# han0110/learn-fhe

Hardware: AMD Instinct MI355X
Metric: NTTs/sec at N=2^14 q~60-bit (higher is better)
Workload: dtype u64

## Files before the change

learn-fhe_amd/csrc/arith.hpp:

```cpp
#pragma once
#include <type_traits>

#include "dev_arith.hpp"

namespace fhe {

#define FHE_GLOBAL __attribute__((address_space(1)))
template <class T>
__device__ __forceinline__ const FHE_GLOBAL T *as_global(const T *p) {
    return (const FHE_GLOBAL T *)p;
}
#define FHE_CONST __attribute__((address_space(4)))
template <class T>
__device__ __forceinline__ const FHE_CONST T *as_const(const T *p) {
    return (const FHE_CONST T *)p;
}

#define FHE_HEADER_KERNEL static __attribute__((unused)) __global__

template <int I, int END, typename F>
__device__ __forceinline__ void static_for(F &&f) {
    if constexpr (I < END) {
        f(std::integral_constant<int, I>{});
        static_for<I + 1, END>(f);
// ... 162 lines not shown
    static __device__ __forceinline__ TwRaw fetch(const K &k, int idx) {
        const FHE_CONST PmRaw *p = (INV ? k.twi : k.tw) + idx;
        TwRaw r;
        r.x = p->x; r.y = p->y;
        return r;
    }
    static __device__ __forceinline__ TwReg prep(const TwRaw &r) { return PmTw{r.x, r.x << (63 - B), r.y}; }
    static __host__ __device__ __forceinline__ PmTw split(u64 w) {
        PmTw t;
        t.wl = (unsigned)(w & ((u64(1) << (B - 31)) - 1));
        t.wlp = t.wl << (63 - B);
        t.wh = (unsigned)(w >> (B - 31));
        return t;
    }
    static __device__ __forceinline__ K make(const ModDesc &D, int log_n_total, int pb, int prefix) {
        K k;
        k.m.q = D.q; k.m.q2 = 2 * D.q; k.m.q4 = 4 * D.q;
        k.m.c = D.pm_c; k.m.c2 = 2 * D.pm_c;
        k.tw = (const FHE_CONST PmRaw *)D.tww; k.twi = (const FHE_CONST PmRaw *)D.twwi;
        k.ninv = split(pb ? 1 : D.ninv[log_n_total]);
        k.ninv_w = split(D.ninv_w[log_n_total]);
        k.pb = pb; k.prefix = prefix;
        return k;
    }
    static __device__ __forceinline__ u64 fold1(u64 x, const PmK &m) {
        const unsigned hi = (unsigned)(x >> 32), h = hi >> (B - 32);
        const u64 base = ((u64)(hi & (unsigned)(MASK >> 32)) << 32) | (unsigned)x;
        return (u64)h * m.c + base;
    }
    static __device__ __forceinline__ u64 mulvar(u64 x, u64 y, const K &k) { return pm_mul<B>(x, split(y), k.m); }
    static __device__ __forceinline__ void ct(u64 &X, u64 &Y, const TwReg &w, const K &k) {
        const u64 t = pm_mul<B>(Y, w, k.m);
        const u64 x = X;
        X = x + t;
        Y = x - t + k.m.q2;
    }
    template <int PH>
    static __device__ __forceinline__ void gs(u64 &X, u64 &Y, const TwReg &w, const K &k) {
        const u64 s = X + Y;
        const u64 d = X - Y + (PH ? k.m.q4 : k.m.q2);
        X = s;
        Y = pm_mul<B>(d, w, k.m);
    }
    static constexpr bool GS_FOLDS = true;
    static constexpr int GS_SPAN = 0;
    template <int PH = 1>
    static __device__ __forceinline__ void gs_last_scaled(u64 &X, u64 &Y, const K &k) {
        const u64 s = X + Y, d = X - Y + k.m.q4;
        X = csub(pm_mul<B>(s, k.ninv, k.m), k.m.q);
        Y = csub(pm_mul<B>(d, k.ninv_w, k.m), k.m.q);
    }
    template <int PH = 1>
    static __device__ __forceinline__ void gs_last_plain(u64 &X, u64 &Y, const PmTw &w, const K &k) {
        const u64 s = X + Y, d = X - Y + k.m.q4;
        X = csub(fold1(s, k.m), k.m.q);
        Y = csub(pm_mul<B>(d, w, k.m), k.m.q);
    }
    static constexpr int CT_LAYERS = ((1 << (63 - B)) + 1) / 2 > 64 ? 64 : ((1 << (63 - B)) + 1) / 2;
    static constexpr bool PASS_FOLD = true;
    static __device__ constexpr bool ct_fold_at(int) { return false; }
    static __device__ __forceinline__ u64 gs_fold(u64 x, const K &k) { return fold1(x, k.m); }
    static __device__ __forceinline__ u64 fold(u64 x, const K &k) { return fold1(x, k.m); }
    static __device__ __forceinline__ u64 canon_fwd(u64 x, const K &k) { return csub(fold1(x, k.m), k.m.q); }
    static __device__ __forceinline__ u64 finish_inv(u64 x, const K &k) { return csub(pm_mul<B>(x, k.ninv, k.m), k.m.q); }
    static constexpr int MAC_TERMS = B <= 54 ? 32 : B == 55 ? 16 : B == 56 ? 8 : 3;
    struct MacAcc { u64 v, u; };
    static __device__ __forceinline__ MacAcc mac_zero() { return MacAcc{0, 0}; }
    static __device__ __forceinline__ u64 mac_in(u64 x, const K &) { return x; }
    static __device__ __forceinline__ MacAcc mac(MacAcc acc, u64 xin, u64 kval, int term, const K &k, const Barrett &) {
        const unsigned wl = (unsigned)kval;
        const PmTw w{wl, wl << (63 - B), (unsigned)(kval >> 32)};
        u64 v, u;
        pm_mul_vu<B>(xin, w, v, u);
        acc.v += v; acc.u += u;
        if ((term % MAC_TERMS) == MAC_TERMS - 1) acc = MacAcc{pm_reduce_vu<B>(acc.v, acc.u, k.m), 0};
        return acc;
    }
    static __device__ __forceinline__ u64 mac_finish(MacAcc acc, const K &k) { return pm_reduce_vu<B>(acc.v, acc.u, k.m); }
};

struct DsK {
    u64 q, q2, q4;
    unsigned c, c2, pw;
};

template <int B>
struct ArithDS {
    typedef u64 Elem;
    static constexpr u64 MASK = (u64(1) << B) - 1;
    static constexpr int SPLIT = B - 31;
    typedef uint4 TwRaw;
    typedef uint4 TwReg;
    struct K {
        DsK m;
        const FHE_CONST uint4 *tw, *twi;
        uint4 ninv, ninv_w;
        int pb, prefix;
        const FHE_CONST uint4 *tw3i;
        unsigned tw3_stride;
    };
    static constexpr int PREFETCH = 4;
    static __host__ __device__ __forceinline__ uint4 split(u64 w, u64 q) {
        const u64 w1 = (u64)((((unsigned __int128)w) << 32) % q);
        const u64 lo = (u64(1) << SPLIT) - 1;
        return uint4{(unsigned)(w & lo), (unsigned)(w >> SPLIT), (unsigned)(w1 & lo), (unsigned)(w1 >> SPLIT)};
    }
    template <bool INV>
    static __device__ __forceinline__ TwRaw fetch(const K &k, int idx) {
        const FHE_CONST uint4 *p = (INV ? k.twi : k.tw) + idx;
        TwRaw r;
        r.x = p->x; r.y = p->y; r.z = p->z; r.w = p->w;
        return r;
    }
    static __device__ __forceinline__ TwReg prep(const TwRaw &r) { return r; }
    static __device__ __forceinline__ K make(const ModDesc &D, int log_n_total, int pb, int prefix) {
        K k;
        k.m.q = D.q; k.m.q2 = 2 * D.q; k.m.q4 = 4 * D.q;
        k.m.c = D.pm_c; k.m.c2 = 2 * D.pm_c; k.m.pw = D.ds_pow;
        k.tw = as_const(D.twd); k.twi = as_const(D.twdi);
        k.ninv = pb ? D.ds_one : D.ds_ninv[log_n_total];
        k.ninv_w = D.ds_ninv_w[log_n_total];
        k.pb = pb; k.prefix = prefix;
        k.tw3i = as_const(D.twd3i); k.tw3_stride = D.twd3_stride;
        return k;
    }
    static __device__ __forceinline__ u64 mul_raw(u64 y, const uint4 &w, const DsK &m) {
        const unsigned y0 = (unsigned)y, y1 = (unsigned)(y >> 32);
        const u64 s1 = (u64)w.y * y0 + (u64)w.w * y1;
        const u64 s0 = (u64)w.x * y0 + (u64)w.z * y1;
        const u64 v = (u64)(unsigned)s1 * m.pw + s0;
        return (u64)(unsigned)(s1 >> 32) * m.c2 + v;
    }
    static __device__ __forceinline__ u64 fold1(u64 x, const DsK &m) {
        const unsigned hi = (unsigned)(x >> 32), h = hi >> (B - 32);
        const u64 base = ((u64)(hi & (unsigned)(MASK >> 32)) << 32) | (unsigned)x;
        return (u64)h * m.c + base;
    }
    static __device__ __forceinline__ u64 mul(u64 y, const uint4 &w, const DsK &m) { return fold1(mul_raw(y, w, m), m); }
    static __device__ __forceinline__ u64 mulvar(u64 x, u64 y, const K &k) {
        return pm_mul<B>(x, ArithPM<B>::split(y), PmK{k.m.q, k.m.q2, k.m.q4, k.m.c, k.m.c2});
    }
    static __device__ __forceinline__ void ct(u64 &X, u64 &Y, const TwReg &w, const K &k) {
        const u64 t = mul(Y, w, k.m);
        const u64 x = X;
        X = x + t;
        Y = x + k.m.q2 - t;
    }
    static constexpr int CT_LAYERS = 64;
    static constexpr bool PASS_FOLD = false;
    static constexpr int CT_SPAN = B >= 64 - 2 ? 1 : (((1 << (64 - B)) - 2) / 2 > 64 ? 64 : ((1 << (64 - B)) - 2) / 2);
    static __device__ constexpr bool ct_fold_at(int layer) { return layer > 0 && layer % CT_SPAN == 0; }
    template <int PH>
    static __device__ __forceinline__ void gs(u64 &X, u64 &Y, const TwReg &w, const K &k) {
        static_assert(PH < 64 - B - 1, "sums overflow");
        const u64 s = X + Y;
        const u64 d = X + (k.m.q2 << PH) - Y;
        X = s;
        Y = mul(d, w, k.m);
    }
    static constexpr bool GS_FOLDS = true;
    static constexpr int GS_SPAN = 64 - B - 1 > 8 ? 8 : 64 - B - 1;
    template <int PH = 1>
    static __device__ __forceinline__ void gs_last_scaled(u64 &X, u64 &Y, const K &k) {
        const u64 s = X + Y, d = X + (k.m.q2 << PH) - Y;
        X = csub(mul(s, k.ninv, k.m), k.m.q);
        Y = csub(mul(d, k.ninv_w, k.m), k.m.q);
    }
    template <int PH = 1>
    static __device__ __forceinline__ void gs_last_plain(u64 &X, u64 &Y, const TwReg &w, const K &k) {
        const u64 s = X + Y, d = X + (k.m.q2 << PH) - Y;
        X = csub(fold1(s, k.m), k.m.q);
        Y = csub(mul(d, w, k.m), k.m.q);
    }
    static __device__ __forceinline__ u64 gs_fold(u64 x, const K &k) { return fold1(x, k.m); }
    static __device__ __forceinline__ u64 fold(u64 x, const K &k) { return fold1(x, k.m); }
    static __device__ __forceinline__ u64 canon_fwd(u64 x, const K &k) { return csub(fold1(x, k.m), k.m.q); }
    static __device__ __forceinline__ u64 finish_inv(u64 x, const K &k) { return csub(mul(x, k.ninv, k.m), k.m.q); }
    typedef typename ArithPM<B>::MacAcc MacAcc;
    static constexpr int MAC_TERMS = ArithPM<B>::MAC_TERMS;
    static __device__ __forceinline__ PmK pmk(const K &k) { return PmK{k.m.q, k.m.q2, k.m.q4, k.m.c, k.m.c2}; }
    static __device__ __forceinline__ MacAcc mac_zero() { return MacAcc{0, 0}; }
    static __device__ __forceinline__ u64 mac_in(u64 x, const K &) { return x; }
    static __device__ __forceinline__ MacAcc mac(MacAcc acc, u64 xin, u64 kval, int term, const K &k, const Barrett &) {
        const unsigned wl = (unsigned)kval;
        const PmTw w{wl, wl << (63 - B), (unsigned)(kval >> 32)};
        u64 v, u;
        pm_mul_vu<B>(xin, w, v, u);
        acc.v += v; acc.u += u;
        if ((term % MAC_TERMS) == MAC_TERMS - 1) acc = MacAcc{pm_reduce_vu<B>(acc.v, acc.u, pmk(k)), 0};
        return acc;
    }
    static __device__ __forceinline__ u64 mac_finish(MacAcc acc, const K &k) { return pm_reduce_vu<B>(acc.v, acc.u, pmk(k)); }
};

#define FHE_SCHED_FENCE() asm volatile("" ::: "memory")

template <int L0_, int R_, int l_, int REP0_, int NREP_, int STRIDE_, bool SHARED_, int REP_SHIFT_ = 0>
struct Unit {
    static constexpr int L0 = L0_, R = R_, l = l_, REP0 = REP0_, NREP = NREP_, STRIDE = STRIDE_, REP_SHIFT = REP_SHIFT_;
    static constexpr bool SHARED = SHARED_;
    static constexpr int NT = (SHARED_ ? 1 : NREP_) << l_;
    static constexpr int half = 1 << (R_ - 1 - l_);
};

#ifdef FHE_LAB_ABLATE
template <class A, class = void> struct tw_skip_mask { static constexpr unsigned value = 0; };
template <class A> struct tw_skip_mask<A, decltype((void)A::SKIP_MASK)> { static constexpr unsigned value = A::SKIP_MASK; };
#endif

template <class A, bool INV, class U, int NTW>
__device__ __forceinline__ void tw_load(typename A::TwRaw (&raw)[NTW], int top, const typename A::K &k) {
    static_assert(U::NT <= NTW, "twiddle buffer too small for this unit");
#pragma unroll
    for (int rr = 0; rr < (U::SHARED ? 1 : U::NREP); ++rr)
#pragma unroll
        for (int b = 0; b < (1 << U::l); ++b) {
            const int tp = U::SHARED ? top : (top | ((U::REP0 + rr) << U::REP_SHIFT));
            const int idx = (1 << (U::L0 + U::l + k.pb)) + ((((k.prefix << U::L0) | tp)) << U::l) + b;
#ifdef FHE_LAB_ABLATE
            if constexpr ((tw_skip_mask<A>::value >> (U::L0 + U::l)) & 1) { raw[(rr << U::l) | b] = A::fake(k, idx); continue; }
#endif
            raw[(rr << U::l) | b] = A::template fetch<INV>(k, idx);
        }
}

template <class A, class U, int NTW, int E>
__device__ __forceinline__ void ct_apply(typename A::Elem (&x)[E], const typename A::TwRaw (&raw)[NTW], const typename A::K &k) {
    if constexpr ((U::l > 0 && U::l % A::CT_LAYERS == 0) || A::ct_fold_at(U::L0 + U::l)) {
#pragma unroll
        for (int rr = 0; rr < U::NREP; ++rr)
#pragma unroll
            for (int r = 0; r < (1 << U::R); ++r) x[(U::REP0 + rr) * U::STRIDE + r] = A::fold(x[(U::REP0 + rr) * U::STRIDE + r], k);
    }
    if constexpr (U::SHARED) {
#pragma unroll
        for (int b = 0; b < (1 << U::l); ++b) {
            const typename A::TwReg w = A::prep(raw[b]);
#pragma unroll
            for (int rr = 0; rr < U::NREP; ++rr)
#pragma unroll
                for (int j = 0; j < U::half; ++j) {
                    const int o = (U::REP0 + rr) * U::STRIDE + b * 2 * U::half + j;
                    A::ct(x[o], x[o + U::half], w, k);
                }
        }
    } else {
#pragma unroll
        for (int rr = 0; rr < U::NREP; ++rr)
#pragma unroll
            for (int b = 0; b < (1 << U::l); ++b) {
                const typename A::TwReg w = A::prep(raw[(rr << U::l) | b]);
#pragma unroll
                for (int j = 0; j < U::half; ++j) {
                    const int o = (U::REP0 + rr) * U::STRIDE + b * 2 * U::half + j;
                    A::ct(x[o], x[o + U::half], w, k);
                }
            }
    }
}

template <class A, class U, int GSTEP = -1, int NTW, int E>
__device__ __forceinline__ void gs_apply(typename A::Elem (&x)[E], const typename A::TwRaw (&raw)[NTW], const typename A::K &k) {
    constexpr bool GLOBAL = GSTEP >= 0 && A::GS_SPAN > 0;
    constexpr int step = U::R - 1 - U::l, PH = GLOBAL ? GSTEP % (A::GS_SPAN > 0 ? A::GS_SPAN : 1) : (step & 1);
    constexpr bool FOLD = A::GS_FOLDS && (GLOBAL ? PH == A::GS_SPAN - 1 : (PH == 1 || step == U::R - 1));
    static_for<0, (U::SHARED ? (1 << U::l) : U::NREP)>([&](auto oc) {
        constexpr int outer = decltype(oc)::value;
        static_for<0, (U::SHARED ? U::NREP : (1 << U::l))>([&](auto ic) {
            constexpr int inner = decltype(ic)::value;
            constexpr int b = U::SHARED ? outer : inner, rr = U::SHARED ? inner : outer;
            const typename A::TwReg w = A::prep(raw[U::SHARED ? b : ((rr << U::l) | b)]);
#pragma unroll
            for (int j = 0; j < U::half; ++j) {
                const int o = (U::REP0 + rr) * U::STRIDE + b * 2 * U::half + j;
                A::template gs<PH>(x[o], x[o + U::half], w, k);
                if constexpr (FOLD) x[o] = A::gs_fold(x[o], k);
            }
        });
    });
}

template <class A, int L0, int R, int OFF, int E>
__device__ __forceinline__ void ct_net(typename A::Elem (&x)[E], int top, const typename A::K &k) {
    static_for<0, R>([&](auto lc) {
        constexpr int l = decltype(lc)::value;
        typedef Unit<L0, R, l, 1, 1, OFF, true> U;
        if constexpr (l > 0) FHE_SCHED_FENCE();
        typename A::TwRaw raw[1 << l];
        tw_load<A, false, U>(raw, top, k);
        ct_apply<A, U>(x, raw, k);
    });
}

template <class A, int L0, int R, int OFF, int E>
__device__ __forceinline__ void gs_net(typename A::Elem (&x)[E], int top, const typename A::K &k) {
    static_for<0, R>([&](auto sc) {
        constexpr int l = R - 1 - decltype(sc)::value;
        typedef Unit<L0, R, l, 1, 1, OFF, true> U;
        if constexpr (l < R - 1) FHE_SCHED_FENCE();
        typename A::TwRaw raw[1 << l];
        tw_load<A, true, U>(raw, top, k);
        gs_apply<A, U>(x, raw, k);
    });
}

}
```

learn-fhe_amd/csrc/ntt14w.hpp:

```cpp
#pragma once
#include <type_traits>
#include "ntt_kernels.hpp"

namespace fhe {
namespace w14 {

constexpr int WSLOTS = 1088;
template <int R0> constexpr int threads() { return 64 << R0; }
template <int R0> constexpr size_t lds_bytes() { return (size_t(1) << R0) * WSLOTS * 8; }
constexpr int THREADS = threads<3>();
constexpr size_t LDS_BYTES = lds_bytes<3>();

__device__ __forceinline__ void wave_sync() {
    __builtin_amdgcn_wave_barrier();
    asm volatile("" ::: "memory");
}
#ifndef W14_XCHG_PRIO
#define W14_XCHG_PRIO 0
#endif
#if W14_XCHG_PRIO
#define W14_PRIO_UP() __builtin_amdgcn_s_setprio(3)
#define W14_PRIO_DOWN() __builtin_amdgcn_s_setprio(0)
#else
#define W14_PRIO_UP()
#define W14_PRIO_DOWN()
#endif

template <class A, class = void> struct w14_old_deal { static constexpr bool value = false; };
template <class A> struct w14_old_deal<A, decltype((void)A::W14_OLD_DEAL)> { static constexpr bool value = true; };
template <class A, int R0>
__device__ __host__ constexpr bool w14_pairs() {
    return R0 <= 3 && !w14_old_deal<A>::value;
}

#ifdef NTT14_STAMPS
__device__ unsigned long long g_stamps[4096][16];
#define STAMP_DECL unsigned long long stamps_[12]
#define STAMP_ENTRY() unsigned long long entry_; asm volatile("s_memrealtime %0\n\ts_waitcnt lgkmcnt(0)" : "=s"(entry_)::"memory")
#define STAMP_ENTRY_ARG , entry_
#define STAMP_ENTRY_PARAM , unsigned long long entry_
#define STAMP(i) asm volatile("s_memtime %0\n\ts_waitcnt lgkmcnt(0)" : "=s"(stamps_[i])::"memory")
#define STAMP_REAL(i) asm volatile("s_memrealtime %0\n\ts_waitcnt lgkmcnt(0)" : "=s"(stamps_[i])::"memory")
#define STAMP_FLUSH()                                                                       \
    do {                                                                                    \
        if (threadIdx.x == 0 && blockIdx.x < 4096)                                          \
            for (int i_ = 0; i_ < 12; ++i_) g_stamps[blockIdx.x][i_] = stamps_[i_];        \
        if (threadIdx.x == 0 && blockIdx.x < 4096) {                                        \
            unsigned hw_, xcc_;                                                             \
            asm volatile("s_getreg_b32 %0, hwreg(HW_REG_HW_ID)" : "=s"(hw_));               \
            asm volatile("s_getreg_b32 %0, hwreg(HW_REG_XCC_ID)" : "=s"(xcc_));             \
            g_stamps[blockIdx.x][12] = ((unsigned long long)xcc_ << 32) | hw_;              \
            g_stamps[blockIdx.x][13] = entry_;                                              \
        }                                                                                   \
    } while (0)
#else
#define STAMP_DECL
#define STAMP_ENTRY()
#define STAMP_ENTRY_ARG
#define STAMP_ENTRY_PARAM
#define STAMP(i)
#define STAMP_REAL(i)
#define STAMP_FLUSH()
#endif


#ifdef W14_LAB_NO_BARRIER
#define W14_SYNC() wave_sync()
#else
#define W14_SYNC() __syncthreads()
#endif

template <int R0, bool PAIRS>
__device__ __forceinline__ void xchg_01(u64 (&x)[32], int t, int w, u64 *lds) {
    constexpr int PB = 5 - R0, NLOW = 1 << (PB - 1);
    u64 *wp = lds + (PAIRS ? 2 * t : t), *rp = lds + (w << 10) + (t & 63);
    u64 y[32];
    W14_PRIO_UP();
#pragma unroll
    for (int h = 0; h < 2; ++h) {
        if constexpr (PAIRS) {
#pragma unroll
            for (int lo = 0; lo < NLOW / 2; ++lo)
#pragma unroll
                for (int n = 0; n < (1 << R0); ++n) {
                    const int r = ((((h * (NLOW / 2)) | lo) << 1) << R0) | n;
                    *reinterpret_cast<ulonglong2 *>(wp + ((n << 10) | (lo << (7 + R0)))) = make_ulonglong2(x[r], x[r + (1 << R0)]);
                }
        } else {
#pragma unroll
            for (int lo = 0; lo < NLOW; ++lo)
#pragma unroll
                for (int n = 0; n < (1 << R0); ++n) wp[(n << 10) | (lo << (10 - (PB - 1)))] = x[((((h << (PB - 1)) | lo)) << R0) | n];
        }
        W14_SYNC();
#pragma unroll
        for (int m = 0; m < 16; ++m) {
            const int n4 = (h << 3) | (m >> 1), s = m & 1;
            y[(s << 4) | n4] = rp[m << 6];
        }
        W14_SYNC();
    }
    W14_PRIO_DOWN();
#pragma unroll
    for (int r = 0; r < 32; ++r) x[r] = y[r];
}

template <int R0, bool PAIRS>
__device__ __forceinline__ void xchg_10(u64 (&x)[32], int t, int w, u64 *lds) {
    constexpr int PB = 5 - R0, NLOW = 1 << (PB - 1);
    u64 *rp = lds + (PAIRS ? 2 * t : t), *wp = lds + (w << 10) + (t & 63);
    u64 y[32];
    W14_PRIO_UP();
    W14_SYNC();
#pragma unroll
    for (int h = 0; h < 2; ++h) {
// ... 117 lines not shown
    return W14_P3_REFILL < 0 ? std::is_same<typename A::TwRaw, uint4>::value : W14_P3_REFILL != 0;
}

template <class A>
struct Tw7 {
    typename A::TwRaw l0[1], l1[2], l2[4];
};
template <class A, bool INV, int R0, int AB>
__device__ __forceinline__ void tw7_load(Tw7<A> &b, int t3, const typename A::K &k) {
    tw_load<A, INV, P3<R0, 0, AB>>(b.l0, t3, k);
    tw_load<A, INV, P3<R0, 1, AB>>(b.l1, t3, k);
    tw_load<A, INV, P3<R0, 2, AB>>(b.l2, t3, k);
}

template <int R0, bool PAIRS>
__device__ __forceinline__ void load_p0(u64 (&x)[32], const u64 *__restrict__ g, int t) {
#pragma unroll
    for (int r = 0; r < 32; ++r) {
        const int n = r & ((1 << R0) - 1), pass = r >> R0;
#ifdef W14_ABLATE_NO_GLOBAL
        x[r] = (u64)(t + r) * 0x9E3779B97F4A7C15ull >> 5;
#else
        if constexpr (PAIRS) {
            if (pass & 1) continue;
            const ulonglong2 v = *reinterpret_cast<const ulonglong2 *>(g + ((n << 11) | ((pass >> 1) << (7 + R0)) | (t << 1)));
            x[r] = v.x; x[r + (1 << R0)] = v.y;
        } else {
            x[r] = g[(n << 11) | (pass << (6 + R0)) | t];
        }
#endif
    }
}
template <int AB>
__device__ __forceinline__ void load_p3(u64 (&x)[32], const u64 *__restrict__ src) {
#pragma unroll
    for (int j = 0; j < 8; j += 2) {
        const ulonglong2 v = *reinterpret_cast<const ulonglong2 *>(src + (AB << 9) + j);
        x[AB * 8 + j] = v.x; x[AB * 8 + j + 1] = v.y;
    }
}
template <class A, int AB>
__device__ __forceinline__ void load_mul_p3(u64 (&x)[32], const u64 *__restrict__ src, const u64 *__restrict__ mul, const typename A::K &k) {
#pragma unroll
    for (int j = 0; j < 8; j += 2) {
        const ulonglong2 v = *reinterpret_cast<const ulonglong2 *>(src + (AB << 9) + j);
        const ulonglong2 m = *reinterpret_cast<const ulonglong2 *>(mul + (AB << 9) + j);
        x[AB * 8 + j] = A::mulvar(v.x, m.x, k); x[AB * 8 + j + 1] = A::mulvar(v.y, m.y, k);
    }
}

template <class A, int AB>
__device__ __forceinline__ void store_p3(u64 (&x)[32], u64 *__restrict__ dst_wave, int lane, u64 *wl, const typename A::K &k) {
    ulonglong2 *wr = reinterpret_cast<ulonglong2 *>(wl + 8 * lane + (lane & ~1));
    const ulonglong2 *rd = reinterpret_cast<const ulonglong2 *>(wl + 2 * lane + 2 * (lane >> 3));
#pragma unroll
    for (int j = 0; j < 4; ++j) {
        ulonglong2 v;
        v.x = A::canon_fwd(x[AB * 8 + 2 * j], k);
        v.y = A::canon_fwd(x[AB * 8 + 2 * j + 1], k);
        wr[j] = v;
    }
    wave_sync();
#pragma unroll
    for (int kk = 0; kk < 4; ++kk) {
        const ulonglong2 v = rd[72 * kk];
        x[AB * 8 + 2 * kk] = v.x; x[AB * 8 + 2 * kk + 1] = v.y;
    }
    wave_sync();
#pragma unroll
    for (int kk = 0; kk < 4; ++kk) {
        ulonglong2 v;
        v.x = x[AB * 8 + 2 * kk]; v.y = x[AB * 8 + 2 * kk + 1];
#ifdef W14_ABLATE_NO_GLOBAL
        if (v.x == 0xdeadbeefcafef00dull)
#endif
        *reinterpret_cast<ulonglong2 *>(dst_wave + (AB << 9) + 128 * kk + 2 * lane) = v;
    }
}

template <class A, int R0, bool KEEP = false>
__device__ __forceinline__ void fwd_one(u64 (&x)[32], u64 *__restrict__ g, const typename A::K &k, u64 *lds, u64 *wl,
                                        const int t, const int lane, const int w STAMP_ENTRY_PARAM) {
    typedef typename A::TwRaw Tw;
    STAMP_DECL;
    STAMP_REAL(10);
    STAMP(0);
    {
        Tw a0[1], a1[2], a2[4], a3[8];
        tw_load<A, false, P0<R0, 0>>(a0, 0, k);
        if constexpr (R0 >= 2) tw_load<A, false, P0<R0, (R0 >= 2 ? 1 : 0)>>(a1, 0, k);
        if constexpr (R0 >= 3) tw_load<A, false, P0<R0, (R0 >= 3 ? 2 : 0)>>(a2, 0, k);
        if constexpr (R0 == 4) tw_load<A, false, P0<R0, (R0 == 4 ? 3 : 0)>>(a3, 0, k);
        STAMP(1);
        FHE_SCHED_FENCE();
        ct_apply<A, P0<R0, 0>>(x, a0, k);
        if constexpr (R0 >= 2) {
            FHE_SCHED_FENCE();
            ct_apply<A, P0<R0, (R0 >= 2 ? 1 : 0)>>(x, a1, k);
        }
        if constexpr (R0 >= 3) {
            FHE_SCHED_FENCE();
            ct_apply<A, P0<R0, (R0 >= 3 ? 2 : 0)>>(x, a2, k);
        }
        if constexpr (R0 == 4) {
            FHE_SCHED_FENCE();
            ct_apply<A, P0<R0, (R0 == 4 ? 3 : 0)>>(x, a3, k);
        }
    }
    FHE_SCHED_FENCE();
    Tw b0[1], b1[2], b2[4], b3[8];
    tw_load<A, false, P1<R0, 0>>(b0, w, k); tw_load<A, false, P1<R0, 1>>(b1, w, k); tw_load<A, false, P1<R0, 2>>(b2, w, k); tw_load<A, false, P1<R0, 3>>(b3, w, k);
    STAMP(2);
    xchg_01<R0, w14_pairs<A, R0>()>(x, t, w, lds);
    STAMP(3);
    if constexpr (A::PASS_FOLD) {
#pragma unroll
        for (int r = 0; r < 32; ++r) x[r] = A::fold(x[r], k);
    }
    FHE_SCHED_FENCE();
    ct_apply<A, P1<R0, 0>>(x, b0, k);
    FHE_SCHED_FENCE();
    ct_apply<A, P1<R0, 1>>(x, b1, k);
    FHE_SCHED_FENCE();
    ct_apply<A, P1<R0, 2>>(x, b2, k);
    FHE_SCHED_FENCE();
    ct_apply<A, P1<R0, 3>>(x, b3, k);
    FHE_SCHED_FENCE();
    const int t2 = (w << 4) | (lane >> 2), t3 = (w << 8) | lane;
    Tw c0[1], c1[2], c2[4], c3[8];
    tw_load<A, false, P2<R0, 0>>(c0, t2, k); tw_load<A, false, P2<R0, 1>>(c1, t2, k); tw_load<A, false, P2<R0, 2>>(c2, t2, k);
    STAMP(4);
    xchg_12(x, lane, wl);
    STAMP(5);
    if constexpr (A::PASS_FOLD) {
#pragma unroll
        for (int r = 0; r < 32; ++r) x[r] = A::fold(x[r], k);
    }
    FHE_SCHED_FENCE();
    ct_apply<A, P2<R0, 0>>(x, c0, k);
    FHE_SCHED_FENCE();
    ct_apply<A, P2<R0, 1>>(x, c1, k);
    FHE_SCHED_FENCE();
    tw_load<A, false, P2<R0, 3>>(c3, t2, k);
    ct_apply<A, P2<R0, 2>>(x, c2, k);
    FHE_SCHED_FENCE();
    ct_apply<A, P2<R0, 3>>(x, c3, k);
    FHE_SCHED_FENCE();
    Tw7<A> d[2];
    tw7_load<A, false, R0, 0>(d[0], t3, k);
    STAMP(6);
    xchg_23(x, lane, wl);
    STAMP(7);
    if constexpr (A::PASS_FOLD) {
#pragma unroll
        for (int r = 0; r < 32; ++r) x[r] = A::fold(x[r], k);
    }
    u64 *dst_wave = g + (w << 11);
    static_for<0, 4>([&](auto abc) {
        constexpr int ab = decltype(abc)::value;
        FHE_SCHED_FENCE();
        ct_apply<A, P3<R0, 0, ab>>(x, d[ab & 1].l0, k);
        ct_apply<A, P3<R0, 1, ab>>(x, d[ab & 1].l1, k);
        FHE_SCHED_FENCE();
        if constexpr (ab < 3) tw7_load<A, false, R0, (ab < 3 ? ab + 1 : 3)>(d[(ab + 1) & 1], t3, k);
        ct_apply<A, P3<R0, 2, ab>>(x, d[ab & 1].l2, k);
        FHE_SCHED_FENCE();
        if constexpr (KEEP) {
#pragma unroll
            for (int j = 0; j < 8; ++j) x[ab * 8 + j] = A::canon_fwd(x[ab * 8 + j], k);
        } else {
            store_p3<A, ab>(x, dst_wave, lane, wl, k);
        }
    });
    STAMP(8);
#ifdef NTT14_STAMPS
    asm volatile("s_waitcnt vmcnt(0)" ::: "memory");
#endif
    STAMP(9);
    STAMP_REAL(11);
    STAMP_FLUSH();
}

template <class A>
__device__ __host__ constexpr bool w14_p3_diag() {
#ifdef W14_NO_DIAG
    return false;
#else
    return std::is_same<typename A::TwRaw, uint4>::value;
#endif
}

template <class A, int R0, int AB>
__device__ __forceinline__ int p3_blk(int t3, const typename A::K &k) {
    return (1 << (R0 + 8 + k.pb)) + ((k.prefix << (R0 + 8)) | t3 | (AB << 6));
}
template <class A, int R0, int AB>
__device__ __forceinline__ void p3_diag_load(uint4 (&e)[7], int t3, const typename A::K &k) {
    const int blk = p3_blk<A, R0, AB>(t3, k);
#pragma unroll
    for (int p = 0; p < 7; ++p) {
        const FHE_CONST uint4 *q = k.tw3i + size_t(p) * k.tw3_stride + blk;
        e[p] = uint4{q->x, q->y, q->z, q->w};
    }
}
template <class A, int R0, int AB, int NEXT>
__device__ __forceinline__ void p3_diag_apply(u64 (&x)[32], uint4 (&e)[7], const uint4 &ci, const uint4 &cj, const uint4 &cij, int t3,
                                              const typename A::K &k) {
    const auto &m = k.m;
    u64 *v = x + 8 * AB;
    const u64 s0 = v[0] + v[1], t0 = v[0] + m.q2 - v[1];
    const u64 s1 = v[2] + v[3], t1 = A::mul(v[2] + m.q2 - v[3], ci, m);
    const u64 s2 = v[4] + v[5], t2 = A::mul(v[4] + m.q2 - v[5], cj, m);
    const u64 s3 = v[6] + v[7], t3v = A::mul(v[6] + m.q2 - v[7], cij, m);
    const u64 u0 = s0 + s1, e0 = s0 + m.q4 - s1;
    const u64 u1 = t0 + t1, e1 = t0 + m.q2 - t1;
    const u64 u2 = s2 + s3, e2 = A::mul(s2 + m.q4 - s3, ci, m);
    const u64 u3 = t2 + t3v, e3 = A::mul(t2 + m.q2 - t3v, ci, m);
    const int blk = NEXT >= 0 ? p3_blk<A, R0, (NEXT >= 0 ? NEXT : 0)>(t3, k) : 0;
    auto refill = [&](int p) {
        if constexpr (NEXT >= 0) {
            const FHE_CONST uint4 *q = k.tw3i + size_t(p) * k.tw3_stride + blk;
            e[p] = uint4{q->x, q->y, q->z, q->w};
        }
    };
    v[0] = A::fold1(u0 + u2, m);
    v[1] = A::mul(u1 + u3, e[0], m); refill(0);
    v[2] = A::mul(e0 + e2, e[1], m); refill(1);
    v[3] = A::mul(e1 + e3, e[2], m); refill(2);
    v[4] = A::mul(u0 + m.q4 - u2, e[3], m); refill(3);
    v[5] = A::mul(u1 + m.q4 - u3, e[4], m); refill(4);
    v[6] = A::mul(e0 + m.q2 - e2, e[5], m); refill(5);
    v[7] = A::mul(e1 + m.q2 - e3, e[6], m); refill(6);
}

template <class A, bool PFX, int R0>
__device__ __forceinline__ void inv_one(u64 (&x)[32], Tw7<A> (&d)[2], u64 *__restrict__ g, const typename A::K &k, u64 *lds, u64 *wl,
                                        const int t, const int lane, const int w STAMP_ENTRY_PARAM) {
    typedef typename A::TwRaw Tw;
    const int t2 = (w << 4) | (lane >> 2), t3 = (w << 8) | lane;
    STAMP_DECL;
    STAMP_REAL(10);
    STAMP(0);
    constexpr bool REFILL = w14_p3_refill<A>();
    Tw c3[8], c2[4], c1[2], c0[1];
    if constexpr (w14_p3_diag<A>()) {
        uint4(&e)[7] = reinterpret_cast<uint4(&)[7]>(d[0]);
        const uint4 ci = A::template fetch<true>(k, 1), cj = A::template fetch<true>(k, 2), cij = A::template fetch<true>(k, 3);
        FHE_SCHED_FENCE();
        p3_diag_apply<A, R0, 0, 1>(x, e, ci, cj, cij, t3, k);
        FHE_SCHED_FENCE();
        p3_diag_apply<A, R0, 1, 2>(x, e, ci, cj, cij, t3, k);
        FHE_SCHED_FENCE();
        p3_diag_apply<A, R0, 2, 3>(x, e, ci, cj, cij, t3, k);
        FHE_SCHED_FENCE();
// ... 232 lines not shown
```

learn-fhe_amd/csrc/ring_api.hip:

```cpp
#include <hip/hip_runtime.h>
#include <cstdlib>

#include <cstring>
#include <mutex>
#include <new>
#include <set>
#include <utility>

#include "../../include/fhe_ring.h"
#include "api_common.hpp"
#include "ctx.hpp"
#include "dispatch.hpp"
#include "ntt_kernels.hpp"
#include "ntt14w.hpp"

using fhe::u64;

namespace {
int check_transform(const fhe_ctx *ctx, const void *a, size_t n, size_t batch) {
    if (!ctx || !is_pow2(n) || (!a && batch)) return FHE_ERR_INVALID;
    if (n == 1) return FHE_OK;
    int log_n = ilog2(n);
    if (log_n > ctx->s - 1) return FHE_ERR_NO_ROOT;
    if (log_n > ctx->log_cap) return FHE_ERR_UNSUPPORTED;
    return FHE_OK;
}

template <class F>
int with_wave_policy(int pm, F &&f) { return fhe::with_policy<fhe::ArithDS, 60, 54, 55>(pm, f); }
template <class F>
int with_gen_policy(int pm, F &&f) { return fhe::with_policy<fhe::ArithPM, 60, 54, 55>(pm, f); }
template <class F>
int with_mul_policy(int pm, F &&f) { return fhe::with_policy<fhe::ArithDS, 60, 54>(pm, f); }

struct GenShape { int log_e, ppw; };
constexpr GenShape GEN_SHAPE[14] = {{0, 0}, {1, 64}, {2, 64}, {3, 64}, {4, 64}, {3, 16}, {3, 16}, {4, 16}, {4, 16}, {4, 8}, {4, 4}, {4, 2}, {4, 1}, {4, 1}};

template <class A, int LOG_N>
int launch_gen(bool inverse, const fhe::ModDesc *descs, unsigned n_desc, u64 *a, size_t subs, hipStream_t st, fhe::NttIo io) {
    constexpr int LOG_E = GEN_SHAPE[LOG_N].log_e, PPW = GEN_SHAPE[LOG_N].ppw;
    using C = fhe::NttCfg<LOG_N, LOG_E, PPW>;
    const unsigned grid = (unsigned)((subs + PPW - 1) / PPW);
    if (inverse)
        return fhe::launch<fhe::ntt_inv_kernel<A, LOG_N, LOG_E, PPW, false, true>>(grid, C::THREADS, C::LDS_BYTES, st, a, descs, n_desc, (unsigned)subs, 0, io);
    return fhe::launch<fhe::ntt_fwd_kernel<A, LOG_N, LOG_E, PPW, false, false>>(grid, C::THREADS, C::LDS_BYTES, st, a, descs, n_desc, (unsigned)subs, 0, io);
}
template <class A>
int dispatch_gen(bool inv, int log_n, const fhe::ModDesc *d, unsigned nd, u64 *a, size_t subs, hipStream_t st, fhe::NttIo io) {
    auto size = [&](auto ln) { return launch_gen<A, decltype(ln)::value>(inv, d, nd, a, subs, st, io); };
    if constexpr (std::is_same_v<A, fhe::ArithShoup>) return fhe::with_int<1, 2, 3, 4, 5, 6, 7, 8, 9, 10, 11, 12, 13>(log_n, size);
    else return fhe::with_int<10, 11, 12, 13>(log_n, size);
}

inline bool limb_major_disabled() { return fhe::opt(fhe::OPT_NO_LIMB_MAJOR) != 0; }
inline bool wave_local_small_disabled() { return fhe::opt(fhe::OPT_NO_W12) != 0; }
inline size_t several_generations() { return size_t(8) * (size_t)fhe::current_cu_count(); }
template <class... P>
inline bool aligned16(const P *...p) { return ((... | (uintptr_t)p) % 16) == 0; }
inline dim3 grid14(unsigned nd, size_t polys, size_t subs) {
    const bool by_mod = nd > 1 && nd <= 65535 && polys % nd == 0 && subs >= several_generations() && !limb_major_disabled();
    return by_mod ? dim3((unsigned)(subs / nd), nd) : dim3((unsigned)subs);
}
template <auto K, int R0>
int launch_w14(const fhe::ModDesc *d, unsigned nd, u64 *a, size_t subs, int pb, hipStream_t st, fhe::NttIo io) {
    return fhe::launch<K>(grid14(nd, subs >> pb, subs), fhe::w14::threads<R0>(), fhe::w14::lds_bytes<R0>(), st, a, d, nd, (unsigned)subs, pb, io);
}
template <class A, int R0>
int launch14(bool inv, const fhe::ModDesc *d, unsigned nd, u64 *a, size_t subs, int pb, hipStream_t st, fhe::NttIo io) {
    if (!aligned16(a, io.mul, io.dst2)) return FHE_ERR_INVALID;
    if constexpr (R0 <= 3) {
        if (!inv && !aligned16(io.src, io.src2, io.src3, io.src4)) return FHE_ERR_INVALID;
    }
    return fhe::with_bool(pb != 0, [&](auto pfx) {
        constexpr bool PFX = decltype(pfx)::value;
        if (!inv) return launch_w14<fhe::ntt14w_fwd_kernel<A, PFX, R0>, R0>(d, nd, a, subs, pb, st, io);
        return fhe::with_bool(io.mul != nullptr, [&](auto mul) {
            return launch_w14<fhe::ntt14w_inv_kernel<A, PFX, decltype(mul)::value, R0>, R0>(d, nd, a, subs, pb, st, io);
        });
    });
}

template <class A, int R0>
int launch_mul14(const fhe::ModDesc *d, unsigned nd, u64 *a, size_t subs, hipStream_t st, fhe::NttIo io) {
    if (!aligned16(a, io.mul)) return FHE_ERR_INVALID;
    return launch_w14<fhe::ntt14w_mul_kernel<A, R0>, R0>(d, nd, a, subs, 0, st, io);
}

int sub_transform(bool inv, const fhe::ModDesc *d, unsigned nd, u64 *a, int log_n, size_t subs, int pb, int pm, hipStream_t st, fhe::NttIo io) {
    if (pb && log_n != 14) return FHE_ERR_UNSUPPORTED;
    if (log_n == 14 || log_n == 15 || ((log_n == 12 || log_n == 13) && !wave_local_small_disabled()))
        return with_wave_policy(pm, [&](auto pol) {
            using A = typename decltype(pol)::type;
            return fhe::with_int<1, 2, 3, 4>(log_n - 11, [&](auto r0) { return launch14<A, decltype(r0)::value>(inv, d, nd, a, subs, pb, st, io); });
        });
    return with_gen_policy(log_n < 10 ? 0 : pm, [&](auto pol) {
        return dispatch_gen<typename decltype(pol)::type>(inv, log_n, d, nd, a, subs, st, io);
    });
}
int sub_fwd(const fhe::ModDesc *d, unsigned nd, u64 *a, int log_n, size_t subs, int pb, int pm, hipStream_t st, fhe::NttIo io) {
    return sub_transform(false, d, nd, a, log_n, subs, pb, pm, st, io);
}
int sub_inv(const fhe::ModDesc *d, unsigned nd, u64 *a, int log_n, size_t subs, int pb, int pm, hipStream_t st, fhe::NttIo io) {
    return sub_transform(true, d, nd, a, log_n, subs, pb, pm, st, io);
}

}

namespace fhe {

int ntt_fwd_multi(const ModDesc *descs, unsigned n_desc, u64 *a, int log_n, size_t batch, hipStream_t st, int pm, NttIo io) {
    if (io.mul) return FHE_ERR_INVALID;
    if (log_n <= 15) return sub_fwd(descs, n_desc, a, log_n, batch, 0, pm, st, io);
// ... 362 lines not shown
```

Before: 14.35 million.

## Use lazy-reduction CT butterflies with compile-time fold schedule in N=2^14 forward NTT

Introduces a lazy Cooley-Tukey butterfly for the double-split pseudo-Mersenne arithmetic. The X input is folded into the multiply accumulation and Y is formed as 2x + K*q - r, so most per-butterfly folds are skipped. A constexpr schedule proves bounds and inserts a fold only on the layers where values would overflow 64 bits. The wave NTT14 forward path uses it by default. It also recomputes the lane id via mbcnt for phase 3 and adds sched barriers every few butterflies, which trades fewer ALU ops for wider intermediate ranges and changed scheduling.

```diff
diff --git a/learn-fhe_amd/csrc/arith.hpp b/learn-fhe_amd/csrc/arith.hpp
--- a/learn-fhe_amd/csrc/arith.hpp
+++ b/learn-fhe_amd/csrc/arith.hpp
@@ -268,7 +268,55 @@
 struct DsK {
     u64 q, q2, q4;
     unsigned c, c2, pw;
-};
+    u64 qk;
+};
+
+template <int B>
+struct DsLazy {
+    typedef unsigned __int128 u128;
+    static constexpr int BITS = B, MAX_LAYERS = 16;
+    static constexpr u128 CAP = u128(1) << 64;
+    static constexpr u128 CMAX = u128(1) << (B - 33);
+    static constexpr u128 QMIN = (u128(1) << B) - CMAX, QMAX = (u128(1) << B) - 1;
+    static constexpr u128 WORD = (u128(1) << 32) - 1;
+    static constexpr u128 LO = (u128(1) << (B - 31)) - 1, HI = (u128(1) << 31) - 1;
+    static constexpr u128 S1MAX = 2 * HI * WORD, S0MAX = 2 * LO * WORD;
+    static constexpr u128 RMAX = S0MAX + WORD * (LO + 1) + WORD * 2 * CMAX;
+    static constexpr u64 K = (u64)((RMAX + QMIN - 1) / QMIN);
+    static constexpr u128 GROW = RMAX > K * QMAX ? RMAX : K * QMAX;
+    static constexpr u128 IN0 = QMAX - 1;
+    static constexpr u128 fold_max(u128 in) { return ((u128(1) << B) - 1) + (in >> B) * CMAX; }
+    struct Sched {
+        bool fold[MAX_LAYERS];
+        u128 in[MAX_LAYERS + 1];
+        bool ok;
+    };
+    static constexpr Sched make() {
+        Sched s{};
+        s.ok = true;
+        s.in[0] = IN0;
+        for (int l = 0; l < MAX_LAYERS; ++l) {
+            s.fold[l] = s.in[l] + GROW >= CAP;
+            const u128 xf = s.fold[l] ? fold_max(s.in[l]) : s.in[l];
+            s.in[l + 1] = xf + GROW;
+            if (s.in[l + 1] >= CAP) s.ok = false;
+        }
+        return s;
+    }
+    static constexpr Sched SCHED = make();
+    static constexpr bool fold_before(int layer) { return SCHED.fold[layer]; }
+    static constexpr u128 in_max(int layer) { return SCHED.in[layer]; }
+    static constexpr bool canon_ok(int n) { return fold_max(SCHED.in[n]) < 2 * QMIN; }
+    static_assert(B >= 34 && B <= 60, "pseudo-Mersenne widths");
+    static_assert(S1MAX < CAP, "S1 = a1 y0 + b1 y1 carries");
+    static_assert(2 * CMAX <= WORD && K * QMAX < CAP, "2c is a 32-bit multiplier, K q a 64-bit constant");
+    static_assert(K * QMIN >= RMAX, "K q must cover the largest raw product for every admitted q");
+    static_assert(SCHED.ok, "a layer's outputs reach 2^64 even with folded inputs");
+    static_assert(canon_ok(12) && canon_ok(13) && canon_ok(14) && canon_ok(15) && canon_ok(16), "canon_fwd needs more than one subtraction");
+};
+static_assert(DsLazy<60>::K == 7 && !DsLazy<60>::fold_before(0) && !DsLazy<60>::fold_before(1) && DsLazy<60>::fold_before(2) &&
+              !DsLazy<60>::fold_before(3) && DsLazy<60>::fold_before(4) && !DsLazy<60>::fold_before(13) && DsLazy<60>::fold_before(14), "60 bits");
+static_assert(DsLazy<55>::K == 7 && !DsLazy<55>::fold_before(15) && DsLazy<54>::K == 7 && !DsLazy<54>::fold_before(15), "54 / 55 bits");
 
 template <int B>
 struct ArithDS {
@@ -303,6 +351,8 @@
         K k;
         k.m.q = D.q; k.m.q2 = 2 * D.q; k.m.q4 = 4 * D.q;
         k.m.c = D.pm_c; k.m.c2 = 2 * D.pm_c; k.m.pw = D.ds_pow;
+        k.m.qk = Lazy::K * D.q;
+        asm("" : "+s"(k.m.qk));
         k.tw = as_const(D.twd); k.twi = as_const(D.twdi);
         k.ninv = pb ? D.ds_one : D.ds_ninv[log_n_total];
         k.ninv_w = D.ds_ninv_w[log_n_total];
@@ -310,14 +360,15 @@
         k.tw3i = as_const(D.twd3i); k.tw3_stride = D.twd3_stride;
         return k;
     }
-    static __device__ __forceinline__ u64 mul_raw(u64 y, const uint4 &w, const DsK &m) {
+    typedef DsLazy<B> Lazy;
+    static __host__ __device__ __forceinline__ u64 mul_raw(u64 y, const uint4 &w, const DsK &m, u64 add = 0) {
         const unsigned y0 = (unsigned)y, y1 = (unsigned)(y >> 32);
         const u64 s1 = (u64)w.y * y0 + (u64)w.w * y1;
-        const u64 s0 = (u64)w.x * y0 + (u64)w.z * y1;
+        const u64 s0 = ((u64)w.x * y0 + add) + (u64)w.z * y1;
         const u64 v = (u64)(unsigned)s1 * m.pw + s0;
         return (u64)(unsigned)(s1 >> 32) * m.c2 + v;
     }
-    static __device__ __forceinline__ u64 fold1(u64 x, const DsK &m) {
+    static __host__ __device__ __forceinline__ u64 fold1(u64 x, const DsK &m) {
         const unsigned hi = (unsigned)(x >> 32), h = hi >> (B - 32);
         const u64 base = ((u64)(hi & (unsigned)(MASK >> 32)) << 32) | (unsigned)x;
         return (u64)h * m.c + base;
@@ -331,6 +382,13 @@
         const u64 x = X;
         X = x + t;
         Y = x + k.m.q2 - t;
+    }
+    template <bool FOLDX>
+    static __host__ __device__ __forceinline__ void ct_lazy(u64 &X, u64 &Y, const TwReg &w, const DsK &m) {
+        const u64 x = FOLDX ? fold1(X, m) : X;
+        const u64 r = mul_raw(Y, w, m, x);
+        X = r;
+        Y = ((x << 1) + m.qk) - r;
     }
     static constexpr int CT_LAYERS = 64;
     static constexpr bool PASS_FOLD = false;
@@ -445,6 +503,26 @@
     }
 }
 
+template <class A, class U, int NTW, int E>
+__device__ __forceinline__ void ct_apply_lazy(typename A::Elem (&x)[E], const typename A::TwRaw (&raw)[NTW], const typename A::K &k) {
+    constexpr bool FOLDX = A::Lazy::fold_before(U::L0 + U::l);
+    constexpr int LAZY_GROUP = 4;
+    static_for<0, (U::SHARED ? (1 << U::l) : U::NREP)>([&](auto oc) {
+        constexpr int outer = decltype(oc)::value;
+        static_for<0, (U::SHARED ? U::NREP : (1 << U::l))>([&](auto ic) {
+            constexpr int inner = decltype(ic)::value;
+            constexpr int b = U::SHARED ? outer : inner, rr = U::SHARED ? inner : outer;
+            const typename A::TwReg w = A::prep(raw[U::SHARED ? b : ((rr << U::l) | b)]);
+#pragma unroll
+            for (int j = 0; j < U::half; ++j) {
+                const int o = (U::REP0 + rr) * U::STRIDE + b * 2 * U::half + j;
+                A::template ct_lazy<FOLDX>(x[o], x[o + U::half], w, k.m);
+                if ((j + 1) % LAZY_GROUP == 0 || j + 1 == U::half) __builtin_amdgcn_sched_barrier(0);
+            }
+        });
+    });
+}
+
 template <class A, class U, int GSTEP = -1, int NTW, int E>
 __device__ __forceinline__ void gs_apply(typename A::Elem (&x)[E], const typename A::TwRaw (&raw)[NTW], const typename A::K &k) {
     constexpr bool GLOBAL = GSTEP >= 0 && A::GS_SPAN > 0;
diff --git a/learn-fhe_amd/csrc/ntt14w.hpp b/learn-fhe_amd/csrc/ntt14w.hpp
--- a/learn-fhe_amd/csrc/ntt14w.hpp
+++ b/learn-fhe_amd/csrc/ntt14w.hpp
@@ -31,6 +31,25 @@
 template <class A, int R0>
 __device__ __host__ constexpr bool w14_pairs() {
     return R0 <= 3 && !w14_old_deal<A>::value;
+}
+
+template <class A, class = void> struct w14_has_lazy { static constexpr bool value = false; };
+template <class A> struct w14_has_lazy<A, std::void_t<typename A::Lazy>> { static constexpr bool value = true; };
+template <class A, class = void> struct w14_eager_ct { static constexpr bool value = false; };
+template <class A> struct w14_eager_ct<A, decltype((void)A::W14_EAGER_CT)> { static constexpr bool value = true; };
+template <class A>
+__device__ __host__ constexpr bool w14_lazy() {
+    return w14_has_lazy<A>::value && !w14_eager_ct<A>::value;
+}
+template <class A, bool KEEP>
+__device__ __host__ constexpr bool w14_lazy_fwd() {
+    if constexpr (w14_lazy<A>()) return !KEEP || A::Lazy::BITS == 60;
+    else return false;
+}
+template <bool LAZY, class A, class U, int NTW, int E>
+__device__ __forceinline__ void w14_ct(typename A::Elem (&x)[E], const typename A::TwRaw (&raw)[NTW], const typename A::K &k) {
+    if constexpr (LAZY) ct_apply_lazy<A, U>(x, raw, k);
+    else ct_apply<A, U>(x, raw, k);
 }
 
 #ifdef NTT14_STAMPS
@@ -314,6 +333,8 @@
 __device__ __forceinline__ void fwd_one(u64 (&x)[32], u64 *__restrict__ g, const typename A::K &k, u64 *lds, u64 *wl,
                                         const int t, const int lane, const int w STAMP_ENTRY_PARAM) {
     typedef typename A::TwRaw Tw;
+    constexpr bool LAZY = w14_lazy_fwd<A, KEEP>();
+    if constexpr (LAZY) static_assert(A::Lazy::canon_ok(11 + R0), "lazy outputs of this many layers do not fit canon_fwd");
     STAMP_DECL;
     STAMP_REAL(10);
     STAMP(0);
@@ -325,18 +346,18 @@
         if constexpr (R0 == 4) tw_load<A, false, P0<R0, (R0 == 4 ? 3 : 0)>>(a3, 0, k);
         STAMP(1);
         FHE_SCHED_FENCE();
-        ct_apply<A, P0<R0, 0>>(x, a0, k);
+        w14_ct<LAZY, A, P0<R0, 0>>(x, a0, k);
         if constexpr (R0 >= 2) {
             FHE_SCHED_FENCE();
-            ct_apply<A, P0<R0, (R0 >= 2 ? 1 : 0)>>(x, a1, k);
+            w14_ct<LAZY, A, P0<R0, (R0 >= 2 ? 1 : 0)>>(x, a1, k);
         }
         if constexpr (R0 >= 3) {
             FHE_SCHED_FENCE();
-            ct_apply<A, P0<R0, (R0 >= 3 ? 2 : 0)>>(x, a2, k);
+            w14_ct<LAZY, A, P0<R0, (R0 >= 3 ? 2 : 0)>>(x, a2, k);
         }
         if constexpr (R0 == 4) {
             FHE_SCHED_FENCE();
-            ct_apply<A, P0<R0, (R0 == 4 ? 3 : 0)>>(x, a3, k);
+            w14_ct<LAZY, A, P0<R0, (R0 == 4 ? 3 : 0)>>(x, a3, k);
         }
     }
     FHE_SCHED_FENCE();
@@ -350,15 +371,15 @@
         for (int r = 0; r < 32; ++r) x[r] = A::fold(x[r], k);
     }
     FHE_SCHED_FENCE();
-    ct_apply<A, P1<R0, 0>>(x, b0, k);
-    FHE_SCHED_FENCE();
-    ct_apply<A, P1<R0, 1>>(x, b1, k);
-    FHE_SCHED_FENCE();
-    ct_apply<A, P1<R0, 2>>(x, b2, k);
-    FHE_SCHED_FENCE();
-    ct_apply<A, P1<R0, 3>>(x, b3, k);
-    FHE_SCHED_FENCE();
-    const int t2 = (w << 4) | (lane >> 2), t3 = (w << 8) | lane;
+    w14_ct<LAZY, A, P1<R0, 0>>(x, b0, k);
+    FHE_SCHED_FENCE();
+    w14_ct<LAZY, A, P1<R0, 1>>(x, b1, k);
+    FHE_SCHED_FENCE();
+    w14_ct<LAZY, A, P1<R0, 2>>(x, b2, k);
+    FHE_SCHED_FENCE();
+    w14_ct<LAZY, A, P1<R0, 3>>(x, b3, k);
+    FHE_SCHED_FENCE();
+    const int t2 = (w << 4) | (lane >> 2), t3e = (w << 8) | lane;
     Tw c0[1], c1[2], c2[4], c3[8];
     tw_load<A, false, P2<R0, 0>>(c0, t2, k); tw_load<A, false, P2<R0, 1>>(c1, t2, k); tw_load<A, false, P2<R0, 2>>(c2, t2, k);
     STAMP(4);
@@ -369,19 +390,25 @@
         for (int r = 0; r < 32; ++r) x[r] = A::fold(x[r], k);
     }
     FHE_SCHED_FENCE();
-    ct_apply<A, P2<R0, 0>>(x, c0, k);
-    FHE_SCHED_FENCE();
-    ct_apply<A, P2<R0, 1>>(x, c1, k);
+    w14_ct<LAZY, A, P2<R0, 0>>(x, c0, k);
+    FHE_SCHED_FENCE();
+    w14_ct<LAZY, A, P2<R0, 1>>(x, c1, k);
     FHE_SCHED_FENCE();
     tw_load<A, false, P2<R0, 3>>(c3, t2, k);
-    ct_apply<A, P2<R0, 2>>(x, c2, k);
-    FHE_SCHED_FENCE();
-    ct_apply<A, P2<R0, 3>>(x, c3, k);
-    FHE_SCHED_FENCE();
+    w14_ct<LAZY, A, P2<R0, 2>>(x, c2, k);
+    FHE_SCHED_FENCE();
+    w14_ct<LAZY, A, P2<R0, 3>>(x, c3, k);
+    FHE_SCHED_FENCE();
+    int lane3 = lane, t3 = t3e;
+    if constexpr (LAZY) {
+        lane3 = __builtin_amdgcn_mbcnt_hi(~0u, __builtin_amdgcn_mbcnt_lo(~0u, 0u));
+        asm volatile("" : "+v"(lane3));
+        t3 = (w << 8) | lane3;
+    }
     Tw7<A> d[2];
     tw7_load<A, false, R0, 0>(d[0], t3, k);
     STAMP(6);
-    xchg_23(x, lane, wl);
+    xchg_23(x, lane3, wl);
     STAMP(7);
     if constexpr (A::PASS_FOLD) {
 #pragma unroll
@@ -391,17 +418,17 @@
     static_for<0, 4>([&](auto abc) {
         constexpr int ab = decltype(abc)::value;
         FHE_SCHED_FENCE();
-        ct_apply<A, P3<R0, 0, ab>>(x, d[ab & 1].l0, k);
-        ct_apply<A, P3<R0, 1, ab>>(x, d[ab & 1].l1, k);
+        w14_ct<LAZY, A, P3<R0, 0, ab>>(x, d[ab & 1].l0, k);
+        w14_ct<LAZY, A, P3<R0, 1, ab>>(x, d[ab & 1].l1, k);
         FHE_SCHED_FENCE();
         if constexpr (ab < 3) tw7_load<A, false, R0, (ab < 3 ? ab + 1 : 3)>(d[(ab + 1) & 1], t3, k);
-        ct_apply<A, P3<R0, 2, ab>>(x, d[ab & 1].l2, k);
+        w14_ct<LAZY, A, P3<R0, 2, ab>>(x, d[ab & 1].l2, k);
         FHE_SCHED_FENCE();
         if constexpr (KEEP) {
 #pragma unroll
             for (int j = 0; j < 8; ++j) x[ab * 8 + j] = A::canon_fwd(x[ab * 8 + j], k);
         } else {
-            store_p3<A, ab>(x, dst_wave, lane, wl, k);
+            store_p3<A, ab>(x, dst_wave, lane3, wl, k);
         }
     });
     STAMP(8);
diff --git a/learn-fhe_amd/csrc/ring_api.hip b/learn-fhe_amd/csrc/ring_api.hip
--- a/learn-fhe_amd/csrc/ring_api.hip
+++ b/learn-fhe_amd/csrc/ring_api.hip
@@ -28,6 +28,9 @@
 
 template <class F>
 int with_wave_policy(int pm, F &&f) { return fhe::with_policy<fhe::ArithDS, 60, 54, 55>(pm, f); }
+template <int... Bs>
+constexpr bool lazy_covers_eligible() { return (... && (fhe::DsLazy<Bs>::CMAX >= ((unsigned __int128)1 << (Bs - 33)))); }
+static_assert(lazy_covers_eligible<60, 54, 55>(), "a pseudo-Mersenne eligible modulus outside the lazy butterflies' proof");
 template <class F>
 int with_gen_policy(int pm, F &&f) { return fhe::with_policy<fhe::ArithPM, 60, 54, 55>(pm, f); }
 template <class F>
```

Measured after the change: 14.76 million (median of 6 runs). 1.03x the previous value.
